# PaddlePaddle/PaddleRobotics

Hardware: NVIDIA H100
Metric: env-steps/sec (A1, 4096 envs) (higher is better)
Workload: dtype f32

## Files before the change

paddlerobotics_b200/build.py:

```python
import os
import subprocess

CSRC = os.path.join(os.path.dirname(os.path.abspath(__file__)), "csrc")
LIB = os.path.join(CSRC, "libb2q.so")
SOURCES = ["b2q_api.cu", "b2q_mlp.cu", "b2q_es.cu", "b2q_sac.cu", "b2q_rpm.cu"]
HEADERS = ["b2q_sim.cuh", "b2q_math.cuh", "b2q_host_common.h", "b2q_model_host.h", "b2q_tc.cuh", "../../include/b2q.h", "../../include/b2q_mlp.h", "../../include/b2q_es.h", "../../include/b2q_sac.h", "../../include/b2q_rpm.h", "b2q_mlp_internal.h"]
NVCC_FLAGS = ["-gencode", "arch=compute_90a,code=sm_90a", "-lineinfo", "-O3", "-std=c++17", "-Xcompiler", "-fPIC", "-shared"]


def _stale():
    if not os.path.exists(LIB):
        return True
    t = os.path.getmtime(LIB)
    for f in SOURCES + HEADERS:
        p = os.path.join(CSRC, f)
        if os.path.exists(p) and os.path.getmtime(p) > t:
            return True
    return False


def build(force=False, verbose=False):
    if not force and not _stale():
        return LIB
    srcs = [os.path.join(CSRC, s) for s in SOURCES if os.path.exists(os.path.join(CSRC, s))]
    nvcc = os.environ.get("NVCC", "/usr/local/cuda/bin/nvcc")
    cmd = [nvcc] + NVCC_FLAGS + (["-Xptxas", "-v"] if verbose else []) + ["-o", LIB] + srcs
    subprocess.check_call(cmd)
    return LIB


if __name__ == "__main__":
    import sys
    print(build(force=True, verbose="-v" in sys.argv))
```

paddlerobotics_b200/csrc/b2q_api.cu:

```cuda
#include <cuda_runtime.h>
#include <cstdio>
#include <cstdlib>
#include <new>
#include <string>
#include "b2q_host_common.h"

using namespace b2q;

namespace {

struct WarpComm {
  int k;
  unsigned char* scr;
  __device__ __forceinline__ int leg() const { return k; }
  template <typename T> __device__ __forceinline__ T* scratch() const { return reinterpret_cast<T*>(scr); }
  __device__ __forceinline__ void sync() const { __syncwarp(); }
  __device__ __forceinline__ bool any(bool f) const { return __any_sync(0xffffffffu, f) != 0; }
  template <typename T>
  __device__ __forceinline__ T sum4(T v) const {
    v += __shfl_xor_sync(0xffffffffu, v, 1);
    v += __shfl_xor_sync(0xffffffffu, v, 2);
    return v;
  }
  template <typename T>
  __device__ __forceinline__ T bcast(T v, int f) const { return __shfl_sync(0xffffffffu, v, f, 4); }
};

template <typename T>
__device__ __forceinline__ const Model<T>& stage_model(const Model<T>* g, unsigned char* smem) {
  Model<T>* s = reinterpret_cast<Model<T>*>(smem);
  const uint4* src = reinterpret_cast<const uint4*>(g);
  uint4* dst = reinterpret_cast<uint4*>(s);
  constexpr int NV = (int)((sizeof(Model<T>) + 15) / 16);
  for (int i0 = threadIdx.x; i0 < NV; i0 += 4 * blockDim.x) {
    uint4 v[4];
#pragma unroll
    for (int k = 0; k < 4; k++) { const int i = i0 + k * (int)blockDim.x; if (i < NV) v[k] = __ldg(src + i); }
#pragma unroll
    for (int k = 0; k < 4; k++) { const int i = i0 + k * (int)blockDim.x; if (i < NV) dst[i] = v[k]; }
  }
  __syncthreads();
  return *s;
}

template <typename T>
__device__ __forceinline__ void copy_block(T* __restrict__ dst, const T* stage, int n) {
  constexpr int PER = 16 / (int)sizeof(T);
  if ((((size_t)dst | (size_t)stage) & 15) == 0 && n % PER == 0) {
    uint4* d4 = reinterpret_cast<uint4*>(dst); const uint4* s4 = reinterpret_cast<const uint4*>(stage);
    for (int i = threadIdx.x; i < n / PER; i += blockDim.x) d4[i] = s4[i];
  } else {
    for (int i = threadIdx.x; i < n; i += blockDim.x) dst[i] = stage[i];
  }
}

template <typename T>
__device__ __forceinline__ void emit_obs_block(const Model<T>& md, const T* stage, T* __restrict__ obs, int env0, int rows) {
  const int od = md.obs_dim;
  T* dst = obs + (size_t)env0 * od;
  if (md.obs_identity) { copy_block(dst, stage, rows * OBS_DIM); return; }
  for (int i = threadIdx.x; i < rows * od; i += blockDim.x) { int r = i / od, j = i - r * od; dst[i] = obs_out_elem(md, stage + r * OBS_DIM, j); }
}

template <typename T, int FEAT>
__global__ void __launch_bounds__(128) b2q_step_kernel(Cfg<T> cf, const Model<T>* __restrict__ gm, Buffers<T> B, const T* __restrict__ action, int donef,
                                                       int auto_reset, T* __restrict__ obs, T* __restrict__ reward, uint8_t* __restrict__ done, T* __restrict__ info) {
  extern __shared__ __align__(32) unsigned char smem[];
  const Model<T>& md = stage_model(gm, smem);
  T* stage = reinterpret_cast<T*>(smem + ((sizeof(Model<T>) + 31) & ~size_t(31)));
  int gid = blockIdx.x * blockDim.x + threadIdx.x;
  int env = gid >> 2;
  const int env0 = (blockIdx.x * blockDim.x) >> 2, per_cta = blockDim.x >> 2;
  bool valid = env < B.N;
  const int srow = env0 + (int)(threadIdx.x >> 2);
  if (!valid) env = B.N - 1;
  T* istage0 = stage + (size_t)per_cta * OBS_DIM;
  WarpComm cm{(int)(threadIdx.x & 3), reinterpret_cast<unsigned char*>(istage0 + (size_t)per_cta * INFO_DIM + (size_t)(threadIdx.x >> 2) * scratch_floats(FEAT))};
  T* istage = istage0;
  step_lane<T, FEAT>(cm, cf, md, B, env, valid, action, donef, auto_reset, stage + (ptrdiff_t)(srow - env) * OBS_DIM, reward, done, istage, env0, env0);
  __syncthreads();
  const int rows = min(per_cta, B.N - env0);
  emit_obs_block(md, stage, obs, env0, rows);
  copy_block(info + (size_t)env0 * INFO_DIM, istage, rows * INFO_DIM);
}

template <typename T, int FEAT>
__global__ void __launch_bounds__(128) b2q_settle_kernel(Cfg<T> cf, const Model<T>* __restrict__ gm, Buffers<T> B, const uint8_t* __restrict__ mask) {
  extern __shared__ __align__(32) unsigned char smem[];
  const Model<T>& md = stage_model(gm, smem);
  int gid = blockIdx.x * blockDim.x + threadIdx.x;
  int env = gid >> 2;
  bool valid = env < B.N;
  if (!valid) env = B.N - 1;
  if (mask && !mask[env]) valid = false;
  T* scr0 = reinterpret_cast<T*>(smem + ((sizeof(Model<T>) + 31) & ~size_t(31))) + (size_t)(blockDim.x >> 2) * (OBS_DIM + INFO_DIM);
  WarpComm cm{(int)(threadIdx.x & 3), reinterpret_cast<unsigned char*>(scr0 + (size_t)(threadIdx.x >> 2) * scratch_floats(FEAT))};
  settle_lane<T, FEAT>(cm, cf, md, B, env, valid);
}

template <typename T>
__global__ void __launch_bounds__(128) b2q_reset_kernel(Cfg<T> cf, const Model<T>* __restrict__ gm, Buffers<T> B, const uint8_t* __restrict__ mask, const T* __restrict__ xoff,
                                                        T* __restrict__ obs) {
  extern __shared__ __align__(32) unsigned char smem[];
  const Model<T>& md = stage_model(gm, smem);
  T* stage = reinterpret_cast<T*>(smem + ((sizeof(Model<T>) + 31) & ~size_t(31)));
  int gid = blockIdx.x * blockDim.x + threadIdx.x;
  int env = gid >> 2;
  const int env0 = (blockIdx.x * blockDim.x) >> 2;
  bool valid = env < B.N;
  if (!valid) env = B.N - 1;
  if (mask && !mask[env]) valid = false;
  WarpComm cm{(int)(threadIdx.x & 3), nullptr};
  T* srow = stage + (size_t)(threadIdx.x >> 2) * OBS_DIM;
  reset_lane<T>(cm, cf, md, B, env, valid, obs ? srow : (T*)nullptr, xoff);
  if (obs) {
    __syncwarp();
// ... 279 lines not shown
  else { auto* t = new (std::nothrow) EnvT<double>(); if (!t) return B2Q_ENOMEM; rc = t->init(*cfg); impl = t; }
  if (rc != B2Q_OK) { g_create_err = impl->err; delete impl; return rc; }
  B2QEnv* h = new (std::nothrow) B2QEnv{impl};
  if (!h) { delete impl; return B2Q_ENOMEM; }
  *out = h;
  return B2Q_OK;
}
int b2q_destroy(B2QHandle h) { if (!h) return B2Q_EINVAL; delete h->impl; delete h; return B2Q_OK; }
const char* b2q_last_error(B2QHandle h) { return h ? h->impl->err.c_str() : g_create_err.c_str(); }
int b2q_num_envs(B2QHandle h) { return h ? h->impl->cfg.num_envs : B2Q_EINVAL; }
int b2q_obs_dim(B2QHandle h) { return h ? h->impl->obs_dim : B2Q_EINVAL; }
int b2q_act_dim(B2QHandle h) { return h ? h->impl->act_dim() : B2Q_EINVAL; }
int b2q_info_dim(B2QHandle h) { return h ? B2Q_INFO_DIM : B2Q_EINVAL; }
int b2q_elem_size(B2QHandle h) { return h ? (h->impl->prec ? 8 : 4) : B2Q_EINVAL; }
int b2q_set_dynamics(B2QHandle h, const uint8_t* m, const void* dyn, void* s) { return h ? h->impl->set_dynamics(m, dyn, (cudaStream_t)s) : B2Q_EINVAL; }
int b2q_reset(B2QHandle h, const uint8_t* m, const void* w, const void* b, void* obs, void* s) { return h ? h->impl->reset(m, w, b, nullptr, obs, (cudaStream_t)s) : B2Q_EINVAL; }
int b2q_reset_ex(B2QHandle h, const uint8_t* m, const void* w, const void* b, const void* xoff, void* obs, void* s) {
  return h ? h->impl->reset(m, w, b, xoff, obs, (cudaStream_t)s) : B2Q_EINVAL;
}
int b2q_set_external_force(B2QHandle h, const void* f, void* s) { return h ? h->impl->set_force(f, (cudaStream_t)s) : B2Q_EINVAL; }
int b2q_step(B2QHandle h, const void* a, int donef, void* obs, void* rew, uint8_t* done, void* info, void* s) {
  return h ? h->impl->step(a, donef, obs, rew, done, info, (cudaStream_t)s) : B2Q_EINVAL;
}
int b2q_step_host(B2QHandle h, const void* a, int donef, void* obs, void* rew, uint8_t* done, void* info, void* s) {
  return h ? h->impl->step_host(a, donef, obs, rew, done, info, (cudaStream_t)s) : B2Q_EINVAL;
}
void* b2q_host_alloc(size_t bytes) { void* p = nullptr; return cudaHostAlloc(&p, bytes, cudaHostAllocDefault) == cudaSuccess ? p : nullptr; }
void b2q_host_free(void* p) { if (p) cudaFreeHost(p); }
int b2q_get_state(B2QHandle h, void* out, void* s) { return h ? h->impl->get_state(out, (cudaStream_t)s) : B2Q_EINVAL; }
int b2q_set_state(B2QHandle h, const void* in, void* s) { return h ? h->impl->set_state(in, (cudaStream_t)s) : B2Q_EINVAL; }
int b2q_get_step_count(B2QHandle h, int32_t* out, void* s) { return h ? h->impl->get_step_count(out, (cudaStream_t)s) : B2Q_EINVAL; }
int64_t b2q_launch_count(B2QHandle h) { return h ? h->impl->launches : 0; }

}
```

paddlerobotics_b200/csrc/b2q_sim.cuh:

```cuda
#pragma once
#include "b2q_math.cuh"

namespace b2q {

constexpr int NS = 37;
constexpr int NP = 15;
constexpr int NE = 16;
constexpr int OBS_DIM = 49;
constexpr int INFO_DIM = 56;
constexpr int ETG_H = 20;

template <typename T>
struct alignas(4 * sizeof(T)) P4 {
  T x, y, z, w;
};

template <typename T>
struct LegModel {
  T p1[3];
  T lhip;
  T com[3][3];
  T I[3][6];
  T m[3];
};
template <typename T>
struct Model {
  LegModel<T> leg[4];
  T m0, I0[6];
  T foot_r, l_up, l_low;
  T etg_u[ETG_H][2];
  T base_foot[4][3];
  T etg_mean[12], etg_std[12], etg_istd[12];
  T pose_ori[3];
  T qlo[3], qhi[3];
  T knee_r;
  int obs_dim, obs_identity;
  int obs_src[OBS_DIM];
  T obs_scale[OBS_DIM], obs_shift[OBS_DIM];
};
template <typename T>
struct Cfg {
  T dt; int R; int iters; T erp, warm, margin; int interp; T tau_limit; int settle_steps;
  int filter; T fb0, fb1, fb2, fa1, fa2; int etg; int max_steps;
// ... 91 lines not shown
  const T two_pi = T(6.283185307179586476925286766559);
  T tt = (k == 0 || k == 3) ? t : t + T(0.5) * cf.etg_T2;
  T om = two_pi / cf.etg_T;
  T x0 = cf.etg_amp * m_sin(cf.etg_ph0 + om * tt), x1 = cf.etg_amp * m_sin(cf.etg_ph1 + om * tt);
  T d[3] = {0, 0, 0};
  const T isig = T(1) / cf.etg_sigma_sq;
  T e[4 * NE];
#pragma unroll
  for (int p = 0; p < NE; p++) { P4<T> v = ldp(etg, p, N, env); e[4 * p] = v.x; e[4 * p + 1] = v.y; e[4 * p + 2] = v.z; e[4 * p + 3] = v.w; }
#pragma unroll
  for (int h = 0; h < ETG_H; h++) {
    T dx = x0 - md.etg_u[h][0], dy = x1 - md.etg_u[h][1];
    T r = m_exp(-(dx * dx + dy * dy) * isig);
#pragma unroll
    for (int a = 0; a < 3; a++) d[a] += e[a * ETG_H + h] * r;
  }
#pragma unroll
  for (int a = 0; a < 3; a++) d[a] += e[60 + a];
  const LegModel<T>& lm = md.leg[k];
  T ang[3];
  for (int tries = 0; tries < 200; tries++) {
    V3<T> f = mk<T>(md.base_foot[k][0] + d[0] - lm.p1[0], md.base_foot[k][1] + d[1] - lm.p1[1], md.base_foot[k][2] + d[2] - lm.p1[2]);
    leg_ik(md, f, lm.lhip, ang);
    if (!(m_isnan(ang[0]) || m_isnan(ang[1]) || m_isnan(ang[2]))) break;
    d[0] *= T(0.95); d[1] *= T(0.95); d[2] *= T(0.95);
  }
#pragma unroll
  for (int a = 0; a < 3; a++) act[a] = ang[a] - md.pose_ori[a];
}

constexpr int RPL = 9, NRW = 4 * RPL;
constexpr int SCRATCH_FLOATS = NRW * 6 + 4 * 45 + NRW * 4 + NRW * NRW;
constexpr int SCRATCH_FAST = 272;
B2Q_HD constexpr int scratch_floats(int feat) { return feat ? SCRATCH_FLOATS : SCRATCH_FAST; }
#define JLIM_GAP T(0.06)
template <typename T, class Comm>
B2Q_HD void solve_rows36(const Comm& cm, const Cfg<T>& cf, T mu, const T (*Y)[6] , const T* u , const T* blk45 ,
                         const T* targ , const bool* act , const T* warm , T* lk ) {
  const int k = cm.leg();
  T* sh = cm.template scratch<T>();
  T* Ya = sh; T* blk = sh + NRW * 6; T* vec = blk + 4 * 45; T* W = vec + NRW * 4;
  cm.sync();
  for (int e = 0; e < RPL; e++) {
    const int r = RPL * k + e;
    for (int c = 0; c < 6; c++) Ya[r * 6 + c] = Y[e][c];
    vec[r * 4 + 0] = u[e]; vec[r * 4 + 1] = targ[e]; vec[r * 4 + 2] = act[e] ? T(1) : T(0); vec[r * 4 + 3] = warm[e];
  }
  for (int i = 0; i < 45; i++) blk[k * 45 + i] = blk45[i];
  cm.sync();
  const int grp_row[9] = {6, 7, 8, 0, 3, 1, 2, 4, 5}, grp_par[9] = {-1, -1, -1, -1, -1, 0, 0, 3, 3};
  int idx[NRW], par[NRW], pos_of[NRW], n = 0;
  for (int i = 0; i < NRW; i++) pos_of[i] = -1;
  for (int seg = 0; seg < 5; seg++) {
    const int g0 = seg == 0 ? 0 : seg == 1 ? 3 : seg == 2 ? 4 : seg == 3 ? 5 : 7, g1 = seg == 0 ? 3 : seg == 1 ? 4 : seg == 2 ? 5 : seg == 3 ? 7 : 9;
    for (int f = 0; f < 4; f++)
      for (int g = g0; g < g1; g++) {
        const int r = RPL * f + grp_row[g];
        if (!(vec[r * 4 + 2] > T(0))) continue;
        idx[n] = r; par[n] = grp_par[g] >= 0 ? pos_of[RPL * f + grp_par[g]] : -1; pos_of[r] = n; n++;
      }
  }
  for (int i = 0; i < n; i++) {
    const int r = idx[i];
    if (r / RPL != k) continue;
    for (int j = 0; j < n; j++) {
      const int c = idx[j];
      T acc = T(0);
      for (int q = 0; q < 6; q++) acc += Ya[r * 6 + q] * Ya[c * 6 + q];
      if (c / RPL == k) { const int a = r - RPL * k, b = c - RPL * k; acc += blk[k * 45 + (a >= b ? a * (a + 1) / 2 + b : b * (b + 1) / 2 + a)]; }
      W[i * NRW + j] = acc;
    }
  }
  cm.sync();
  T lam[NRW], uu[NRW];
  for (int i = 0; i < n; i++) lam[i] = vec[idx[i] * 4 + 3];
  for (int i = 0; i < n; i++) { T a = vec[idx[i] * 4 + 0]; for (int j = 0; j < n; j++) a += W[i * NRW + j] * lam[j]; uu[i] = a; }
  for (int it = 0; it < cf.iters; it++) {
    for (int i = 0; i < n; i++) {
      T ln = lam[i] + (vec[idx[i] * 4 + 1] - uu[i]) / W[i * NRW + i];
      if (par[i] >= 0) { T lim = mu * lam[par[i]]; ln = m_min(m_max(ln, -lim), lim); } else ln = m_max(ln, T(0));
      T dl = ln - lam[i]; lam[i] = ln;
      for (int j = 0; j < n; j++) uu[j] += W[j * NRW + i] * dl;
    }
  }
  for (int e = 0; e < RPL; e++) { const int q = pos_of[RPL * k + e]; lk[e] = q >= 0 ? lam[q] : T(0); }
  cm.sync();
}

template <typename T, int FEAT, class Comm>
B2Q_HD void substep(const Comm& cm, const Cfg<T>& cf, const Model<T>& md, const LaneParam<T>& pr, LaneState<T>& s,
                    const T* target, T* tau_out, V3<T> fext = V3<T>{0, 0, 0}, const T* hyb = nullptr ) {
  const int k = cm.leg();
  const LegModel<T>& lm = md.leg[k];
  const T dt = cf.dt, idt = cf.idt;
  R3<T> R = quat_to_R(s.qx, s.qy, s.qz, s.qw);
  V3<T> wB = rotT(R, s.vang), vB = rotT(R, s.vlin), gB = rotT(R, pr.g);

  T tau[3];
#pragma unroll
  for (int j = 0; j < 3; j++) {
    T cmd = target[j];
    if (cf.clip_cmd) cmd = m_min(m_max(cmd, s.q[j] - cf.max_dq), s.q[j] + cf.max_dq);
    T t = T(-1) * (pr.kp[j] * (s.q[j] - cmd)) - pr.kd[j] * (s.qd[j] - T(0));
    if (FEAT && cf.motor_mode == 1) t = target[j];
    if (FEAT && cf.motor_mode == 2) t = T(-1) * (hyb[j] * (s.q[j] - cmd)) - hyb[6 + j] * (s.qd[j] - hyb[3 + j]) + hyb[9 + j];
    if (cf.tau_limit > T(0)) t = m_min(m_max(t, -cf.tau_limit), cf.tau_limit);
    tau[j] = t; tau_out[j] = t;
  }

  LegKin<T> K; leg_kin(md, lm, s.q, K);
  const V3<T> a1 = mk<T>(1, 0, 0), a2 = K.a2;
  V3<T> cL[3]; S3<T> IL[3]; T mL[3];
  {
    const R3<T>* Rs[3] = {&K.R1, &K.R2, &K.R3m};
    const V3<T> ps[3] = {K.p1, K.p2, K.p3};
#pragma unroll
    for (int i = 0; i < 3; i++) {
      cL[i] = ps[i] + rot(*Rs[i], mk<T>(lm.com[i][0], lm.com[i][1], lm.com[i][2]));
      S3<T> Il = {lm.I[i][0], lm.I[i][1], lm.I[i][2], lm.I[i][3], lm.I[i][4], lm.I[i][5]};
// ... 123 lines not shown
  bool act = dist < cf.margin;
  V3<T> t1w = mk<T>(1 - n_w.x * n_w.x, -n_w.x * n_w.y, -n_w.x * n_w.z);
  t1w = t1w * m_rsqrt(dot(t1w, t1w));
  V3<T> t2w = cross(n_w, t1w);
  V3<T> eB[3] = {rotT(R, n_w), rotT(R, t1w), rotT(R, t2w)};
  V3<T> xc = K.toe - eB[0] * md.foot_r;
  T Jk[3][3], u[3], Y[3][6], Wl[3][3];
  {
    V3<T> r1 = cross(a1, xc - K.p1), r2 = cross(a2, xc - K.p2), r3 = cross(a2, xc - K.p3);
#pragma unroll
    for (int e = 0; e < 3; e++) {
      Jk[e][0] = dot(eB[e], r1); Jk[e][1] = dot(eB[e], r2); Jk[e][2] = dot(eB[e], r3);
      V6<T> Jb; Jb.a = cross(xc, eB[e]); Jb.l = eB[e];
      u[e] = dot(Jb.a, wBs) + dot(Jb.l, vBs) + Jk[e][0] * qds[0] + Jk[e][1] * qds[1] + Jk[e][2] * qds[2];
      const T Jba[6] = {Jb.a.x, Jb.a.y, Jb.a.z, Jb.l.x, Jb.l.y, Jb.l.z};
#pragma unroll
      for (int c = 0; c < 6; c++) {
        T g = Jba[c];
#pragma unroll
        for (int j = 0; j < 3; j++) g = m_fma(FD[j][c], -Jk[e][j], g);
        Y[e][c] = g;
      }
      fwd6(S, Li, Y[e]);
    }
#pragma unroll
    for (int e = 0; e < 3; e++) {
      T dj[3];
#pragma unroll
      for (int i = 0; i < 3; i++) dj[i] = D[i][0] * Jk[e][0] + D[i][1] * Jk[e][1] + D[i][2] * Jk[e][2];
#pragma unroll
      for (int e2 = 0; e2 < 3; e2++) Wl[e2][e] = Jk[e2][0] * dj[0] + Jk[e2][1] * dj[1] + Jk[e2][2] * dj[2];
    }
  }
  T lk[3] = {T(0), T(0), T(0)};
  T lkx[6] = {T(0), T(0), T(0), T(0), T(0), T(0)}, Yx[6][6], Jx[6][3];
#pragma unroll
  for (int e = 0; e < 6; e++) {
#pragma unroll
    for (int c = 0; c < 6; c++) Yx[e][c] = T(0);
    Jx[e][0] = Jx[e][1] = Jx[e][2] = T(0);
  }
  bool general = false;
  if constexpr (FEAT != 0) {
    bool need = false;
    T kdist = T(1); V3<T> kn_w = mk<T>(0, 0, 1);
    if (cf.jlim) {
#pragma unroll
      for (int j = 0; j < 3; j++) need = need || (s.q[j] - md.qlo[j] < JLIM_GAP) || (md.qhi[j] - s.q[j] < JLIM_GAP);
    }
    if (cf.knee) {
      V3<T> kw = s.pos + rot(R, K.p3);
      kdist = kw.z - terrain_height(cf, kw.x, kw.y, kn_w) - md.knee_r;
      need = need || (kdist < cf.margin);
    }
    if ((cf.jlim || cf.knee) && cm.any(need)) {
      T Y9[RPL][6], u9[RPL], targ9[RPL], warm9[RPL], blk[45], Jall[RPL][3]; bool act9[RPL];
#pragma unroll
      for (int e = 0; e < 3; e++) {
#pragma unroll
        for (int c = 0; c < 6; c++) Y9[e][c] = Y[e][c];
        u9[e] = u[e]; targ9[e] = T(0); warm9[e] = T(0); act9[e] = act;
        Jall[e][0] = Jk[e][0]; Jall[e][1] = Jk[e][1]; Jall[e][2] = Jk[e][2];
      }
      targ9[0] = dist > T(0) ? -dist * idt : cf.erp * (-dist) * idt; warm9[0] = cf.warm * s.lam_n;
      {
        const bool kact = cf.knee && (kdist < cf.margin);
// ... 25 lines not shown
        fwd6(S, Li, Yx[3 + j]);
        Jx[3 + j][0] = j == 0 ? sj : T(0); Jx[3 + j][1] = j == 1 ? sj : T(0); Jx[3 + j][2] = j == 2 ? sj : T(0);
        u9[6 + j] = sj * qds[j];
        targ9[6 + j] = gap > T(0) ? -gap * idt : cf.erp * (-gap) * idt;
        warm9[6 + j] = cf.warm * s.lam_lim[j];
        act9[6 + j] = cf.jlim && (gap < JLIM_GAP);
      }
#pragma unroll
      for (int e = 0; e < 6; e++) {
#pragma unroll
        for (int c = 0; c < 6; c++) Y9[3 + e][c] = Yx[e][c];
        Jall[3 + e][0] = Jx[e][0]; Jall[3 + e][1] = Jx[e][1]; Jall[3 + e][2] = Jx[e][2];
      }
#pragma unroll
      for (int a = 0; a < RPL; a++) {
        T dj[3];
#pragma unroll
        for (int i = 0; i < 3; i++) dj[i] = D[i][0] * Jall[a][0] + D[i][1] * Jall[a][1] + D[i][2] * Jall[a][2];
#pragma unroll
        for (int b = 0; b <= a; b++) blk[a * (a + 1) / 2 + b] = Jall[b][0] * dj[0] + Jall[b][1] * dj[1] + Jall[b][2] * dj[2];
      }
      T lk9[RPL];
      solve_rows36<T>(cm, cf, pr.mu, Y9, u9, blk, targ9, act9, warm9, lk9);
#pragma unroll
      for (int e = 0; e < 3; e++) lk[e] = lk9[e];
#pragma unroll
      for (int e = 0; e < 6; e++) lkx[e] = lk9[3 + e];
      general = true;
    }
  }
  if (!general) {
  T g[12], Wc[12][12], lam[12];
  {
    T* sh = cm.template scratch<T>();
    T* YT = sh;
    T* vecs = sh + 72;
    T* afs = sh + 120;
    T* Wp = sh + 128;
    const T targ_n = dist > T(0) ? -dist * idt : cf.erp * (-dist) * idt;
    T invo[3];
#pragma unroll
    for (int e = 0; e < 3; e++) {
      T d = Wl[e][e];
#pragma unroll
      for (int c = 0; c < 6; c++) d = m_fma(Y[e][c], Y[e][c], d);
      invo[e] = act ? m_rcp(d) : T(0);
      const int i = 3 * k + e;
#pragma unroll
      for (int c = 0; c < 6; c++) YT[c * 12 + i] = Y[e][c];
      vecs[i] = invo[e]; vecs[12 + i] = u[e]; vecs[24 + i] = e == 0 ? targ_n : T(0);
      vecs[36 + i] = (e == 0 && act) ? cf.warm * s.lam_n : T(0);
    }
    afs[k] = act ? T(1) : T(0);
    cm.sync();
    {
      T Ya[12][6], inv[12];
#pragma unroll
      for (int c = 0; c < 6; c++) {
#pragma unroll
        for (int q = 0; q < 3; q++) {
          const P4<T> v = *reinterpret_cast<const P4<T>*>(YT + c * 12 + 4 * q);
          Ya[4 * q][c] = v.x; Ya[4 * q + 1][c] = v.y; Ya[4 * q + 2][c] = v.z; Ya[4 * q + 3][c] = v.w;
        }
      }
#pragma unroll
      for (int q = 0; q < 3; q++) { const P4<T> v = *reinterpret_cast<const P4<T>*>(vecs + 4 * q); inv[4 * q] = v.x; inv[4 * q + 1] = v.y; inv[4 * q + 2] = v.z; inv[4 * q + 3] = v.w; }
// ... 16 lines not shown
#pragma unroll
          for (int c = 0; c < 6; c++) w = m_fma(Y[e2][c], Y[e][c], w);
          Wp[r * 12 + 3 * k + e2] = (e2 == e) ? T(0) : w * invo[e2];
        }
      }
    }
    cm.sync();
#pragma unroll
    for (int r = 0; r < 12; r++) {
#pragma unroll
      for (int q = 0; q < 3; q++) { const P4<T> v = *reinterpret_cast<const P4<T>*>(Wp + r * 12 + 4 * q); Wc[r][4 * q] = v.x; Wc[r][4 * q + 1] = v.y; Wc[r][4 * q + 2] = v.z; Wc[r][4 * q + 3] = v.w; }
    }
    {
      const P4<T> af = *reinterpret_cast<const P4<T>*>(afs);
      const T actf[4] = {af.x, af.y, af.z, af.w};
      T lw[4];
#pragma unroll
      for (int q = 0; q < 3; q++) {
        const P4<T> iv = *reinterpret_cast<const P4<T>*>(vecs + 4 * q), uv = *reinterpret_cast<const P4<T>*>(vecs + 12 + 4 * q);
        const P4<T> tv = *reinterpret_cast<const P4<T>*>(vecs + 24 + 4 * q), lv = *reinterpret_cast<const P4<T>*>(vecs + 36 + 4 * q);
        g[4 * q] = (tv.x - uv.x) * iv.x; g[4 * q + 1] = (tv.y - uv.y) * iv.y; g[4 * q + 2] = (tv.z - uv.z) * iv.z; g[4 * q + 3] = (tv.w - uv.w) * iv.w;
        lam[4 * q] = lv.x; lam[4 * q + 1] = lv.y; lam[4 * q + 2] = lv.z; lam[4 * q + 3] = lv.w;
      }
#pragma unroll
      for (int f = 0; f < 4; f++) lw[f] = lam[3 * f];
#pragma unroll
      for (int i = 0; i < 12; i++) {
#pragma unroll
        for (int f = 0; f < 4; f++) g[i] = m_fma(Wc[3 * f][i], -lw[f], g[i]);
        if (i % 3 == 0 && !(actf[i / 3] > T(0))) g[i] = T(-1e30);
      }
    }
    cm.sync();
  }
  for (int it = 0; it < cf.iters; it++) {
#pragma unroll
    for (int f = 0; f < 4; f++) {
      const int r = 3 * f;
      T ln = m_max(g[r], T(0));
      T dl = lam[r] - ln; lam[r] = ln;
#pragma unroll
      for (int i = 0; i < 12; i++)
        if (i != r) g[i] = m_fma(Wc[r][i], dl, g[i]);
    }
#pragma unroll
    for (int f = 0; f < 4; f++) {
#pragma unroll
      for (int td = 1; td < 3; td++) {
        const int r = 3 * f + td;
        T lim = pr.mu * lam[3 * f];
        T ln = m_min(m_max(g[r], -lim), lim);
        T dl = lam[r] - ln; lam[r] = ln;
#pragma unroll
        for (int i = 0; i < 12; i++)
          if (i != r) g[i] = m_fma(Wc[r][i], dl, g[i]);
      }
    }
  }
#pragma unroll
  for (int f = 0; f < 4; f++) if (f == k) { lk[0] = lam[3 * f]; lk[1] = lam[3 * f + 1]; lk[2] = lam[3 * f + 2]; }
  }
  s.lam_n = lk[0]; s.contact = lk[0] > T(0); s.lam_lim[0] = lkx[3]; s.lam_lim[1] = lkx[4]; s.lam_lim[2] = lkx[5];
  T z[6];
#pragma unroll
  for (int c = 0; c < 6; c++) z[c] = cm.sum4(Y[0][c] * lk[0] + Y[1][c] * lk[1] + Y[2][c] * lk[2] + (FEAT != 0 ? Yx[0][c] * lkx[0] + Yx[1][c] * lkx[1] + Yx[2][c] * lkx[2] + Yx[3][c] * lkx[3] + Yx[4][c] * lkx[4] + Yx[5][c] * lkx[5] : T(0)));
  bwd6(S, Li, z);
  V6<T> dnu = arr_to_v6(z);
  {
    T jl[3], t[3];
#pragma unroll
    for (int i = 0; i < 3; i++) {
      jl[i] = Jk[0][i] * lk[0] + Jk[1][i] * lk[1] + Jk[2][i] * lk[2];
      if (FEAT != 0) jl[i] += Jx[0][i] * lkx[0] + Jx[1][i] * lkx[1] + Jx[2][i] * lkx[2] + Jx[3][i] * lkx[3] + Jx[4][i] * lkx[4] + Jx[5][i] * lkx[5];
      t[i] = jl[i] - dot6(Fc[i], dnu);
    }
#pragma unroll
    for (int j = 0; j < 3; j++) qds[j] += D[j][0] * t[0] + D[j][1] * t[1] + D[j][2] * t[2];
  }
  wBs = wBs + dnu.a; vBs = vBs + dnu.l;
  s.vang = rot(R, wBs); s.vlin = rot(R, vBs);
#pragma unroll
  for (int j = 0; j < 3; j++) { s.qd[j] = qds[j]; s.q[j] += dt * qds[j]; }
  s.pos = s.pos + s.vlin * dt;
  {
    T wx = s.vang.x, wy = s.vang.y, wz = s.vang.z, th = m_sqrt(wx * wx + wy * wy + wz * wz) * dt;
    T sh, cw; sincos_t(T(0.5) * th, sh, cw);
    T kk = th < T(1e-4) ? T(0.5) - th * th * T(1.0 / 48.0) : sh * m_rcp(th);
    T dx = wx * dt * kk, dy = wy * dt * kk, dz = wz * dt * kk;
    T ox = cw * s.qx + dx * s.qw + dy * s.qz - dz * s.qy;
    T oy = cw * s.qy - dx * s.qz + dy * s.qw + dz * s.qx;
    T oz = cw * s.qz + dx * s.qy - dy * s.qx + dz * s.qw;
    T ow = cw * s.qw - dx * s.qx - dy * s.qy - dz * s.qz;
    T nn = m_rsqrt(ox * ox + oy * oy + oz * oz + ow * ow);
    s.qx = ox * nn; s.qy = oy * nn; s.qz = oz * nn; s.qw = ow * nn;
  }
}

template <typename T> B2Q_HD P4<T> ldp(const P4<T>* base, int pack, int N, int env) { return base[(size_t)pack * N + env]; }
template <typename T> B2Q_HD void stp(P4<T>* base, int pack, int N, int env, T x, T y, T z, T w) {
  P4<T> p; p.x = x; p.y = y; p.z = z; p.w = w; base[(size_t)pack * N + env] = p;
}

template <typename T, class Comm>
B2Q_HD void load_param(const Comm& cm, const Buffers<T>& B, int env, LaneParam<T>& pr) {
  const int k = cm.leg(), N = B.N;
  P4<T> a = ldp(B.param, 0 + k, N, env), b = ldp(B.param, 4 + k, N, env), c = ldp(B.param, 8 + k, N, env);
  P4<T> d = ldp(B.param, 12, N, env), e = ldp(B.param, 13, N, env), g = ldp(B.param, 14, N, env);
  pr.kp[0] = a.x; pr.kp[1] = a.y; pr.kp[2] = a.z; pr.mu = a.w;
  pr.kd[0] = b.x; pr.kd[1] = b.y; pr.kd[2] = b.z; pr.latency = b.w;
  pr.iscale[0] = c.x; pr.iscale[1] = c.y; pr.iscale[2] = c.z;
  pr.mscale[0] = d.x; pr.mscale[1] = d.y; pr.mscale[2] = d.z; pr.m0s = d.w;
  pr.I0s[0] = e.x; pr.I0s[1] = e.y; pr.I0s[2] = e.z;
  pr.g = mk<T>(g.x, g.y, g.z);
}
template <typename T, class Comm>
B2Q_HD void load_state(const Comm& cm, const P4<T>* st, int N, int env, LaneState<T>& s, T* last_action, T* etg_act, int& has_last, V3<T>& rpy0) {
  const int k = cm.leg();
  P4<T> p0 = ldp(st, 0, N, env), p1 = ldp(st, 1, N, env), p2 = ldp(st, 2, N, env), p3 = ldp(st, 3, N, env);
  P4<T> pq = ldp(st, 4 + k, N, env), pd = ldp(st, 8 + k, N, env), pa = ldp(st, 12 + k, N, env), pe = ldp(st, 16 + k, N, env), pr = ldp(st, 20, N, env);
  s.pos = mk<T>(p0.x, p0.y, p0.z); s.qx = p1.x; s.qy = p1.y; s.qz = p1.z; s.qw = p1.w;
  s.vlin = mk<T>(p2.x, p2.y, p2.z); has_last = p2.w > T(0.5);
  s.vang = mk<T>(p3.x, p3.y, p3.z);
  s.q[0] = pq.x; s.q[1] = pq.y; s.q[2] = pq.z; s.lam_n = pq.w;
  s.qd[0] = pd.x; s.qd[1] = pd.y; s.qd[2] = pd.z; s.contact = pq.w > T(0);
  last_action[0] = pa.x; last_action[1] = pa.y; last_action[2] = pa.z; s.lam_lim[0] = pa.w; s.lam_lim[1] = pe.w; s.lam_lim[2] = pd.w;
  etg_act[0] = pe.x; etg_act[1] = pe.y; etg_act[2] = pe.z;
  rpy0 = mk<T>(pr.x, pr.y, pr.z);
}
// ... 131 lines not shown
  if (FEAT && cf.motor_mode == 2) {
#pragma unroll
    for (int j = 0; j < 3; j++) {
      const T* a5 = action + ((size_t)env * 12 + 3 * k + j) * 5;
      target[j] = a5[0]; hyb[j] = a5[1]; hyb[3 + j] = a5[2]; hyb[6 + j] = a5[3]; hyb[9 + j] = a5[4];
    }
  }
  if (cf.filter && !(FEAT && cf.motor_mode == 2)) {
    P4<T> x1 = ldp(B.state, 21 + 4 * k, N, env), x2 = ldp(B.state, 22 + 4 * k, N, env), y1 = ldp(B.state, 23 + 4 * k, N, env), y2 = ldp(B.state, 24 + 4 * k, N, env);
    T ax1[3] = {x1.x, x1.y, x1.z}, ax2[3] = {x2.x, x2.y, x2.z}, ay1[3] = {y1.x, y1.y, y1.z}, ay2[3] = {y2.x, y2.y, y2.z}, yy[3];
#pragma unroll
    for (int j = 0; j < 3; j++) yy[j] = cf.fb0 * target[j] + cf.fb1 * ax1[j] + cf.fb2 * ax2[j] - cf.fa1 * ay1[j] - cf.fa2 * ay2[j];
    if (valid) {
      stp(B.state, 21 + 4 * k, N, env, target[0], target[1], target[2], T(0)); stp(B.state, 22 + 4 * k, N, env, ax1[0], ax1[1], ax1[2], T(0));
      stp(B.state, 23 + 4 * k, N, env, yy[0], yy[1], yy[2], T(0)); stp(B.state, 24 + 4 * k, N, env, ay1[0], ay1[1], ay1[2], T(0));
    }
#pragma unroll
    for (int j = 0; j < 3; j++) target[j] = yy[j];
  }
  const V3<T> start_pos = s.pos;
  T foot0_x;
  {
    LegKin<T> K; leg_kin(md, md.leg[k], s.q, K);
    R3<T> Rb = quat_to_R(s.qx, s.qy, s.qz, s.qw);
    foot0_x = s.pos.x + rot(Rb, K.toe).x;
  }
  int n_lag = pr.latency > T(0) ? (int)(pr.latency / cf.dt) : 0;
  T alpha = pr.latency > T(0) ? (pr.latency - T(n_lag) * cf.dt) / cf.dt : T(0);
  int max_lag = B.Dm * R - 2; if (n_lag > max_lag) { n_lag = max_lag; alpha = T(0); }
  int ia = ((R - 1 - n_lag) % R + R) % R, ma = (n_lag - (R - 1 - ia)) / R;
  int ib = ((R - 2 - n_lag) % R + R) % R, mb = (n_lag + 1 - (R - 1 - ib)) / R;
  const int slot = step % B.Dm;
  T tau[3] = {0, 0, 0};
#pragma unroll 1
  for (int i = 0; i < R; i++) {
    T proc[3];
    if (cf.interp && has_last && !(FEAT && cf.motor_mode == 2)) {
      T lerp = T(i + 1) / T(R);
#pragma unroll
      for (int j = 0; j < 3; j++) proc[j] = last_action[j] + lerp * (target[j] - last_action[j]);
    } else {
#pragma unroll
      for (int j = 0; j < 3; j++) proc[j] = target[j];
    }
    substep<T, FEAT>(cm, cf, md, pr, s, proc, tau, fext, hyb);
    if (valid && i == ia) ring_write(B, slot, 0, k, env, s.q, s.qd, tau);
    if (valid && i == ib) ring_write(B, slot, 1, k, env, s.q, s.qd, tau);
  }
#pragma unroll
  for (int j = 0; j < 3; j++) last_action[j] = target[j];
  has_last = 1;
  T dq[3], dqd[3], dtau[3];
  {
    T aq[3], aqd[3], at[3], bq[3], bqd[3], bt[3];
    ring_read(B, ((step - ma) % B.Dm + B.Dm) % B.Dm, 0, k, env, aq, aqd, at);
    ring_read(B, ((step - mb) % B.Dm + B.Dm) % B.Dm, 1, k, env, bq, bqd, bt);
#pragma unroll
    for (int j = 0; j < 3; j++) {
      dq[j] = (T(1) - alpha) * aq[j] + alpha * bq[j];
      dqd[j] = (T(1) - alpha) * aqd[j] + alpha * bqd[j];
      dtau[j] = (T(1) - alpha) * at[j] + alpha * bt[j];
    }
  }
  step += 1;
  T nz6[6] = {0, 0, 0, 0, 0, 0};
  if (cf.noise_on) {
// ... 61 lines not shown
      if (valid) stp(B.pos_hist, (step - 1) % STUCK_H, N, env, s.pos.x, s.pos.y, s.pos.z, T(0));
      if (step > STUCK_H) {
        T mx = 0, my = 0, mz = 0, vx = 0, vy = 0, vz = 0;
        for (int h = 0; h < STUCK_H; h++) {
          P4<T> ph = ldp(B.pos_hist, h, N, env);
          T dx = ((step - 1) % STUCK_H == h) ? T(0) : ph.x - s.pos.x, dy = ((step - 1) % STUCK_H == h) ? T(0) : ph.y - s.pos.y, dz = ((step - 1) % STUCK_H == h) ? T(0) : ph.z - s.pos.z;
          mx += dx; my += dy; mz += dz; vx += dx * dx; vy += dy * dy; vz += dz * dz;
        }
        const T inv = T(1) / T(STUCK_H);
        mx *= inv; my *= inv; mz *= inv;
        T var = (vx * inv - mx * mx) + (vy * inv - my * my) + (vz * inv - mz * mz);
        stuckf = (var <= T(2e-4) * T(2e-4)) ? T(1) : T(0);
      }
    }
    stuckf = cm.bcast(stuckf, 0);
  }
  bool dn = fall || donef || (cf.max_steps > 0 && step >= cf.max_steps) || (stuckf > T(0));
  if (valid) {
    T* irow = info + (size_t)(env - info_env0) * INFO_DIM;
    if (k == 0) {
      reward[env] = rew; done[env] = dn ? 1 : 0;
      irow[0] = velx; irow[1] = r_torso; irow[2] = r_feet; irow[3] = r_up; irow[4] = r_tau; irow[5] = 0; irow[6] = r_bad; irow[7] = r_fc; irow[8] = r_done;
      irow[9] = nanf > T(0) ? T(1) : T(0); irow[10] = energy; irow[11] = s.pos.z;
      V3<T> wb = rotT(Rb, s.vang);
      irow[36] = rpy.x; irow[37] = rpy.y; irow[38] = rpy.z; irow[39] = wb.x; irow[40] = wb.y; irow[41] = wb.z;
      irow[54] = fall ? T(1) : T(0); irow[55] = T(step);
      B.step_count[env] = step;
    }
#pragma unroll
    for (int j = 0; j < 3; j++) { irow[12 + 3 * k + j] = etg_act[j]; irow[24 + 3 * k + j] = target[j]; irow[42 + 3 * k + j] = s.q[j]; }
    store_state(cm, B.state, N, env, s, last_action, etg_act, has_last, rpy0);
  }
  if (auto_reset) {
    if (dn) reset_lane(cm, cf, md, B, env, valid, orow);
  }
}

}
```

Baseline: 33.78 million.

## Spill contact-solve intermediates to shared scratch and reorder PGS sweep; add region clocks

```diff
diff --git a/paddlerobotics_b200/build.py b/paddlerobotics_b200/build.py
--- a/paddlerobotics_b200/build.py
+++ b/paddlerobotics_b200/build.py
@@ -8,10 +8,10 @@
 NVCC_FLAGS = ["-gencode", "arch=compute_90a,code=sm_90a", "-lineinfo", "-O3", "-std=c++17", "-Xcompiler", "-fPIC", "-shared"]
 
 
-def _stale():
-    if not os.path.exists(LIB):
+def _stale(lib):
+    if not os.path.exists(lib):
         return True
-    t = os.path.getmtime(LIB)
+    t = os.path.getmtime(lib)
     for f in SOURCES + HEADERS:
         p = os.path.join(CSRC, f)
         if os.path.exists(p) and os.path.getmtime(p) > t:
@@ -19,14 +19,14 @@
     return False
 
 
-def build(force=False, verbose=False):
-    if not force and not _stale():
-        return LIB
+def build(force=False, verbose=False, lib=LIB, defines=()):
+    if not force and not _stale(lib):
+        return lib
     srcs = [os.path.join(CSRC, s) for s in SOURCES if os.path.exists(os.path.join(CSRC, s))]
     nvcc = os.environ.get("NVCC", "/usr/local/cuda/bin/nvcc")
-    cmd = [nvcc] + NVCC_FLAGS + (["-Xptxas", "-v"] if verbose else []) + ["-o", LIB] + srcs
+    cmd = [nvcc] + NVCC_FLAGS + ["-D" + d for d in defines] + (["-Xptxas", "-v"] if verbose else []) + ["-o", lib] + srcs
     subprocess.check_call(cmd)
-    return LIB
+    return lib
 
 
 if __name__ == "__main__":
diff --git a/paddlerobotics_b200/csrc/b2q_api.cu b/paddlerobotics_b200/csrc/b2q_api.cu
--- a/paddlerobotics_b200/csrc/b2q_api.cu
+++ b/paddlerobotics_b200/csrc/b2q_api.cu
@@ -9,9 +9,21 @@
 
 namespace {
 
+#ifdef B2Q_REGION_CLOCKS
+__device__ unsigned long long g_region_clocks[RG_COUNT + 1];
+#endif
+
 struct WarpComm {
   int k;
   unsigned char* scr;
+#ifdef B2Q_REGION_CLOCKS
+  mutable long long t0 = 0;
+  __device__ __forceinline__ void region_end(int r) const {
+    const long long t = clock64();
+    if ((threadIdx.x & 31) == 0) atomicAdd(&g_region_clocks[r], (unsigned long long)(t - t0));
+    t0 = t;
+  }
+#endif
   __device__ __forceinline__ int leg() const { return k; }
   template <typename T> __device__ __forceinline__ T* scratch() const { return reinterpret_cast<T*>(scr); }
   __device__ __forceinline__ void sync() const { __syncwarp(); }
@@ -66,6 +78,9 @@
 __global__ void __launch_bounds__(128) b2q_step_kernel(Cfg<T> cf, const Model<T>* __restrict__ gm, Buffers<T> B, const T* __restrict__ action, int donef,
                                                        int auto_reset, T* __restrict__ obs, T* __restrict__ reward, uint8_t* __restrict__ done, T* __restrict__ info) {
   extern __shared__ __align__(32) unsigned char smem[];
+#ifdef B2Q_REGION_CLOCKS
+  const long long t_start = clock64();
+#endif
   const Model<T>& md = stage_model(gm, smem);
   T* stage = reinterpret_cast<T*>(smem + ((sizeof(Model<T>) + 31) & ~size_t(31)));
   int gid = blockIdx.x * blockDim.x + threadIdx.x;
@@ -77,11 +92,18 @@
   T* istage0 = stage + (size_t)per_cta * OBS_DIM;
   WarpComm cm{(int)(threadIdx.x & 3), reinterpret_cast<unsigned char*>(istage0 + (size_t)per_cta * INFO_DIM + (size_t)(threadIdx.x >> 2) * scratch_floats(FEAT))};
   T* istage = istage0;
+#ifdef B2Q_REGION_CLOCKS
+  cm.t0 = t_start;
+#endif
   step_lane<T, FEAT>(cm, cf, md, B, env, valid, action, donef, auto_reset, stage + (ptrdiff_t)(srow - env) * OBS_DIM, reward, done, istage, env0, env0);
   __syncthreads();
   const int rows = min(per_cta, B.N - env0);
   emit_obs_block(md, stage, obs, env0, rows);
   copy_block(info + (size_t)env0 * INFO_DIM, istage, rows * INFO_DIM);
+#ifdef B2Q_REGION_CLOCKS
+  cm.region_end(RG_EPILOGUE);
+  if ((threadIdx.x & 31) == 0) atomicAdd(&g_region_clocks[RG_COUNT], 1ull);
+#endif
 }
 
 template <typename T, int FEAT>
@@ -427,4 +449,16 @@
 int b2q_get_step_count(B2QHandle h, int32_t* out, void* s) { return h ? h->impl->get_step_count(out, (cudaStream_t)s) : B2Q_EINVAL; }
 int64_t b2q_launch_count(B2QHandle h) { return h ? h->impl->launches : 0; }
 
-}
+#ifdef B2Q_REGION_CLOCKS
+int b2q_region_clocks(unsigned long long* out, int zero) {
+  if (!out) return B2Q_EINVAL;
+  if (cudaDeviceSynchronize() != cudaSuccess || cudaMemcpyFromSymbol(out, g_region_clocks, sizeof(g_region_clocks)) != cudaSuccess) return B2Q_ECUDA;
+  if (zero) {
+    const unsigned long long z[RG_COUNT + 1] = {};
+    if (cudaMemcpyToSymbol(g_region_clocks, z, sizeof(z)) != cudaSuccess) return B2Q_ECUDA;
+  }
+  return B2Q_OK;
+}
+#endif
+
+}
diff --git a/paddlerobotics_b200/csrc/b2q_sim.cuh b/paddlerobotics_b200/csrc/b2q_sim.cuh
--- a/paddlerobotics_b200/csrc/b2q_sim.cuh
+++ b/paddlerobotics_b200/csrc/b2q_sim.cuh
@@ -9,6 +9,13 @@
 constexpr int OBS_DIM = 49;
 constexpr int INFO_DIM = 56;
 constexpr int ETG_H = 20;
+
+enum Region { RG_PROLOGUE, RG_BODY, RG_EXCHANGE, RG_SWEEP, RG_APPLY, RG_EPILOGUE, RG_RESET, RG_COUNT };
+#ifdef B2Q_REGION_CLOCKS
+#define B2Q_REGION_END(r) cm.region_end(r)
+#else
+#define B2Q_REGION_END(r) ((void)0)
+#endif
 
 template <typename T>
 struct alignas(4 * sizeof(T)) P4 {
@@ -166,7 +173,8 @@
 constexpr int RPL = 9, NRW = 4 * RPL;
 constexpr int SCRATCH_FLOATS = NRW * 6 + 4 * 45 + NRW * 4 + NRW * NRW;
 constexpr int SCRATCH_FAST = 272;
-B2Q_HD constexpr int scratch_floats(int feat) { return feat ? SCRATCH_FLOATS : SCRATCH_FAST; }
+constexpr int KEEP_FLOATS = 60;
+B2Q_HD constexpr int scratch_floats(int feat) { return feat ? SCRATCH_FLOATS : SCRATCH_FAST + 4 * KEEP_FLOATS + 16; }
 #define JLIM_GAP T(0.06)
 template <typename T, class Comm>
 B2Q_HD void solve_rows36(const Comm& cm, const Cfg<T>& cf, T mu, const T (*Y)[6] , const T* u , const T* blk45 ,
@@ -219,6 +227,27 @@
   }
   for (int e = 0; e < RPL; e++) { const int q = pos_of[RPL * k + e]; lk[e] = q >= 0 ? lam[q] : T(0); }
   cm.sync();
+}
+
+template <typename T>
+B2Q_HD void pgs_sweep(T (&g)[12], T (&lam)[12], const T (&Wc)[12][12], T mu) {
+  constexpr int order[12] = {0, 3, 6, 9, 1, 2, 4, 5, 7, 8, 10, 11};
+#pragma unroll
+  for (int s = 0; s < 12; s++) {
+    const int r = order[s], nx = order[(s + 1) % 12];
+    T ln;
+    if (r % 3 == 0) {
+      ln = m_max(g[r], T(0));
+    } else {
+      const T lim = mu * lam[r - r % 3];
+      ln = m_min(m_max(g[r], -lim), lim);
+    }
+    const T dl = lam[r] - ln; lam[r] = ln;
+    g[nx] = m_fma(Wc[r][nx], dl, g[nx]);
+#pragma unroll
+    for (int i = 0; i < 12; i++)
+      if (i != r && i != nx) g[i] = m_fma(Wc[r][i], dl, g[i]);
+  }
 }
 
 template <typename T, int FEAT, class Comm>
@@ -408,6 +437,24 @@
       for (int e2 = 0; e2 < 3; e2++) Wl[e2][e] = Jk[e2][0] * dj[0] + Jk[e2][1] * dj[1] + Jk[e2][2] * dj[2];
     }
   }
+  if constexpr (FEAT == 0) {
+    T kv[KEEP_FLOATS];
+#pragma unroll
+    for (int i = 0; i < 21; i++) kv[i] = S[i];
+#pragma unroll
+    for (int i = 0; i < 6; i++) kv[21 + i] = Li[i];
+#pragma unroll
+    for (int e = 0; e < 3; e++) { kv[27 + 3 * e] = Jk[e][0]; kv[28 + 3 * e] = Jk[e][1]; kv[29 + 3 * e] = Jk[e][2]; }
+    kv[36] = D[0][0]; kv[37] = D[0][1]; kv[38] = D[0][2]; kv[39] = D[1][1]; kv[40] = D[1][2]; kv[41] = D[2][2];
+#pragma unroll
+    for (int i = 0; i < 3; i++) {
+#pragma unroll
+      for (int c = 0; c < 6; c++) kv[42 + 6 * i + c] = Fa[i][c];
+    }
+    T* kp = cm.template scratch<T>() + SCRATCH_FAST + KEEP_FLOATS * k;
+#pragma unroll
+    for (int q = 0; q < KEEP_FLOATS / 4; q++) { P4<T> v; v.x = kv[4 * q]; v.y = kv[4 * q + 1]; v.z = kv[4 * q + 2]; v.w = kv[4 * q + 3]; *reinterpret_cast<P4<T>*>(kp + 4 * q) = v; }
+  }
   T lk[3] = {T(0), T(0), T(0)};
   T lkx[6] = {T(0), T(0), T(0), T(0), T(0), T(0)}, Yx[6][6], Jx[6][3];
 #pragma unroll
@@ -499,6 +546,7 @@
   if (!general) {
   T g[12], Wc[12][12], lam[12];
   {
+    B2Q_REGION_END(RG_BODY);
     T* sh = cm.template scratch<T>();
     T* YT = sh;
     T* vecs = sh + 72;
@@ -581,33 +629,33 @@
       }
     }
     cm.sync();
-  }
-  for (int it = 0; it < cf.iters; it++) {
-#pragma unroll
-    for (int f = 0; f < 4; f++) {
-      const int r = 3 * f;
-      T ln = m_max(g[r], T(0));
-      T dl = lam[r] - ln; lam[r] = ln;
-#pragma unroll
-      for (int i = 0; i < 12; i++)
-        if (i != r) g[i] = m_fma(Wc[r][i], dl, g[i]);
-    }
-#pragma unroll
-    for (int f = 0; f < 4; f++) {
-#pragma unroll
-      for (int td = 1; td < 3; td++) {
-        const int r = 3 * f + td;
-        T lim = pr.mu * lam[3 * f];
-        T ln = m_min(m_max(g[r], -lim), lim);
-        T dl = lam[r] - ln; lam[r] = ln;
-#pragma unroll
-        for (int i = 0; i < 12; i++)
-          if (i != r) g[i] = m_fma(Wc[r][i], dl, g[i]);
-      }
-    }
-  }
+    B2Q_REGION_END(RG_EXCHANGE);
+  }
+  for (int it = 0; it < cf.iters; it++) pgs_sweep(g, lam, Wc, pr.mu);
+  B2Q_REGION_END(RG_SWEEP);
 #pragma unroll
   for (int f = 0; f < 4; f++) if (f == k) { lk[0] = lam[3 * f]; lk[1] = lam[3 * f + 1]; lk[2] = lam[3 * f + 2]; }
+  }
+  if constexpr (FEAT == 0) {
+    const T* sh = cm.template scratch<T>();
+    const T* kp = sh + SCRATCH_FAST + KEEP_FLOATS * k;
+    T kv[KEEP_FLOATS];
+#pragma unroll
+    for (int q = 0; q < KEEP_FLOATS / 4; q++) { const P4<T> v = *reinterpret_cast<const P4<T>*>(kp + 4 * q); kv[4 * q] = v.x; kv[4 * q + 1] = v.y; kv[4 * q + 2] = v.z; kv[4 * q + 3] = v.w; }
+#pragma unroll
+    for (int i = 0; i < 21; i++) S[i] = kv[i];
+#pragma unroll
+    for (int i = 0; i < 6; i++) Li[i] = kv[21 + i];
+#pragma unroll
+    for (int e = 0; e < 3; e++) { Jk[e][0] = kv[27 + 3 * e]; Jk[e][1] = kv[28 + 3 * e]; Jk[e][2] = kv[29 + 3 * e]; }
+    D[0][0] = kv[36]; D[0][1] = D[1][0] = kv[37]; D[0][2] = D[2][0] = kv[38]; D[1][1] = kv[39]; D[1][2] = D[2][1] = kv[40]; D[2][2] = kv[41];
+#pragma unroll
+    for (int i = 0; i < 3; i++) { Fc[i].a = mk<T>(kv[42 + 6 * i], kv[43 + 6 * i], kv[44 + 6 * i]); Fc[i].l = mk<T>(kv[45 + 6 * i], kv[46 + 6 * i], kv[47 + 6 * i]); }
+#pragma unroll
+    for (int e = 0; e < 3; e++) {
+#pragma unroll
+      for (int c = 0; c < 6; c++) Y[e][c] = sh[c * 12 + 3 * k + e];
+    }
   }
   s.lam_n = lk[0]; s.contact = lk[0] > T(0); s.lam_lim[0] = lkx[3]; s.lam_lim[1] = lkx[4]; s.lam_lim[2] = lkx[5];
   T z[6];
@@ -643,6 +691,7 @@
     T nn = m_rsqrt(ox * ox + oy * oy + oz * oz + ow * ow);
     s.qx = ox * nn; s.qy = oy * nn; s.qz = oz * nn; s.qw = ow * nn;
   }
+  B2Q_REGION_END(RG_APPLY);
 }
 
 template <typename T> B2Q_HD P4<T> ldp(const P4<T>* base, int pack, int N, int env) { return base[(size_t)pack * N + env]; }
@@ -840,6 +889,7 @@
   int ib = ((R - 2 - n_lag) % R + R) % R, mb = (n_lag + 1 - (R - 1 - ib)) / R;
   const int slot = step % B.Dm;
   T tau[3] = {0, 0, 0};
+  B2Q_REGION_END(RG_PROLOGUE);
 #pragma unroll 1
   for (int i = 0; i < R; i++) {
     T proc[3];
@@ -967,8 +1017,12 @@
     store_state(cm, B.state, N, env, s, last_action, etg_act, has_last, rpy0);
   }
   if (auto_reset) {
-    if (dn) reset_lane(cm, cf, md, B, env, valid, orow);
-  }
-}
-
-}
+    if (dn) {
+      B2Q_REGION_END(RG_EPILOGUE);
+      reset_lane(cm, cf, md, B, env, valid, orow);
+      B2Q_REGION_END(RG_RESET);
+    }
+  }
+}
+
+}
```

Result: no change. 34.15 million (median of 6 runs) (+1.1%).
